# Ycblue/TransMIL-DeepGraft

Measured on AMD Instinct MI355X. Metric: slides/sec (fwd+bwd) at N=8192 patches, d=512, higher is better.
Workload: dtype bf16; 1 GPU; TransMIL_feat 2-class, 1 bag N=8192x512 per GPU, train step fwd+CE+bwd+allreduce+Lookahead(RAdam); execution=hipGraph replay of the whole step (one graph per resident bag), global_batch=1, seq_len=8192, parallelism=dp1, accumulate_grad_batches=1

## Files before the change

transmil_deepgraft_amd/csrc/pinv_split.hip:

```cpp
#include "common.h"
#include "a3_combine.h"
#include "../../include/transmil_hip.h"

namespace {

constexpr int NL = 256;
constexpr int MAT = NL * NL;
constexpr int PC = 64 * 128;
constexpr int SLOT = 4 * PC;
constexpr int NSLOT = 3;
constexpr int STAGE_LDS = NSLOT * SLOT;
constexpr int EROW = 68;
constexpr int EPI_LDS = 64 * EROW * 4;
constexpr int MAXJ = 3;
constexpr int NPROD = 8;
constexpr int NTHREADS = 64 * (4 + NPROD);

typedef __attribute__((address_space(3))) void lds_t;
typedef __attribute__((address_space(1))) void glb_t;
typedef __attribute__((address_space(3))) bf16x4 lds_v4;

struct SOp {
  const bf16* p;
  int kr;
  int pad;
};

enum { KIND_PRODUCT = 0, KIND_ABSSUMS = 1 };

struct SJob {
  SOp a[2], b[2];
  int nterms, kind;
  float alpha, diag;
  int alpha_cpow, e1_cpow;
  const void* e1; float e1s; int e1_f32;
  const void* e2; float e2s; int e2_f32;
  void* c; int c_f32; int pad0;
  float* cf;
  bf16* c2; float c2_alpha, c2_diag, c2_e1;
  bf16* c3; float c3_e1; int pad1;
};
TM_DEV const float* job_dotx(const SJob& J) { return (const float*)J.e2; }
TM_DEV float* job_dot_part(const SJob& J) { return J.cf; }

struct SLaunch {
  SJob j[MAXJ];
  int njobs, nbh;
  long long plane;
  const float* maxima;
  const float* X;
  float* sums;
  float* maxima_out;
  A3Combine a3;
#ifdef TM_DIAG
  unsigned long long* stamps;
#endif
};

#ifdef TM_DIAG
unsigned long long* g_split_stamps = nullptr;
#define SPLIT_STAMPS (stamp_out != nullptr)
#else
#define SPLIT_STAMPS false
#endif

TM_DEV unsigned long long stamp() {
  unsigned long long t;
  asm volatile("s_memtime %0\n\ts_waitcnt lgkmcnt(0)" : "=s"(t)::"memory");
  return t;
}
TM_DEV unsigned long long rstamp() {
  unsigned long long t;
  asm volatile("s_memrealtime %0\n\ts_waitcnt lgkmcnt(0)" : "=s"(t)::"memory");
  return t;
}

TM_DEV float powc(float c, int p) { return p == 0 ? 1.f : (p == 1 ? c : c * c); }

TM_DEV float inv_c(const float* maxima, int nbh) {
  typedef const __attribute__((address_space(4))) float cfloat;
  cfloat* m = (cfloat*)(uintptr_t)maxima;
  float mc = -INFINITY, mr = -INFINITY;
  for (int h = 0; h < nbh; ++h) { mc = fmaxf(mc, m[h]); mr = fmaxf(mr, m[nbh + h]); }
  return 1.f / (mc * mr);
}

TM_DEV unsigned lds_off(const void* p) { return (unsigned)(uintptr_t)(const __attribute__((address_space(3))) char*)p; }
template <int OFF> TM_DEV void ds_b128(bf16x8& d, unsigned a) {
  asm volatile("ds_read_b128 %0, %1 offset:%2" : "=v"(d) : "v"(a), "n"(OFF) : "memory");
}
template <int OFF> TM_DEV void ds_tr(bf16x4& d, unsigned a) {
  asm volatile("ds_read_b64_tr_b16 %0, %1 offset:%2" : "=v"(d) : "v"(a), "n"(OFF) : "memory");
}
template <int N> TM_DEV void wait_lgkm() {
  asm volatile("s_waitcnt lgkmcnt(%0)" ::"n"(N) : "memory");
  __builtin_amdgcn_sched_barrier(0);
}

TM_DEV unsigned kc_addr(int ob, int s, int lane) {
  const int r = ob + (lane & 31), c = 2 * s + (lane >> 5);
  return r * 128 + ((c ^ ((r >> 1) & 7)) << 4);
}
TM_DEV unsigned kr_addr(int ob, int lane) {
  const int g = lane >> 4, q = (lane & 15) >> 2, p = lane & 3;
  const int o = ob + (g & 1) * 16 + 4 * p;
  const int k = 8 * (g >> 1) + q;
  const int c = o >> 3, half = (o >> 2) & 1;
  return k * 128 + ((c ^ (((k >> 1) & 1) << 2)) << 4) + half * 8;
}

struct Frag { bf16x8 h, l; };
TM_DEV bf16x8 join(const bf16x4& a, const bf16x4& b) { return (bf16x8){a[0], a[1], a[2], a[3], b[0], b[1], b[2], b[3]}; }

template <int KR, int S, int PL>
TM_DEV void read_op(Frag& f, unsigned krbase, const unsigned (&kc)[4]) {
  if constexpr (KR) {
    bf16x4 a, b, c, d;
    ds_tr<PL * PC + S * 2048>(a, krbase);
    ds_tr<PL * PC + S * 2048 + 512>(b, krbase);
    ds_tr<(PL + 1) * PC + S * 2048>(c, krbase);
    ds_tr<(PL + 1) * PC + S * 2048 + 512>(d, krbase);
    f.h = join(a, b);
    f.l = join(c, d);
  } else {
    ds_b128<PL * PC>(f.h, kc[S]);
    ds_b128<(PL + 1) * PC>(f.l, kc[S]);
  }
}

template <int AKR, int BKR>
TM_DEV void chunk_mma(f32x16& acc, unsigned sb, unsigned akr, unsigned bkr, const unsigned (&akc0)[4],
                      const unsigned (&bkc0)[4]) {
  constexpr int RS = (AKR ? 4 : 2) + (BKR ? 4 : 2);
  unsigned akc[4], bkc[4];
#pragma unroll
  for (int s = 0; s < 4; ++s) { akc[s] = akc0[s] + sb; bkc[s] = bkc0[s] + sb; }
  const unsigned ab = akr + sb, bb = bkr + sb;
  Frag a[2], b[2];
  read_op<AKR, 0, 0>(a[0], ab, akc); read_op<BKR, 0, 2>(b[0], bb, bkc);
  read_op<AKR, 1, 0>(a[1], ab, akc); read_op<BKR, 1, 2>(b[1], bb, bkc);
  wait_lgkm<RS>();
  acc = __builtin_amdgcn_mfma_f32_32x32x16_bf16(a[0].l, b[0].h, acc, 0, 0, 0);
  acc = __builtin_amdgcn_mfma_f32_32x32x16_bf16(a[0].h, b[0].l, acc, 0, 0, 0);
  acc = __builtin_amdgcn_mfma_f32_32x32x16_bf16(a[0].h, b[0].h, acc, 0, 0, 0);
  read_op<AKR, 2, 0>(a[0], ab, akc); read_op<BKR, 2, 2>(b[0], bb, bkc);
  wait_lgkm<RS>();
  acc = __builtin_amdgcn_mfma_f32_32x32x16_bf16(a[1].l, b[1].h, acc, 0, 0, 0);
  acc = __builtin_amdgcn_mfma_f32_32x32x16_bf16(a[1].h, b[1].l, acc, 0, 0, 0);
  acc = __builtin_amdgcn_mfma_f32_32x32x16_bf16(a[1].h, b[1].h, acc, 0, 0, 0);
  read_op<AKR, 3, 0>(a[1], ab, akc); read_op<BKR, 3, 2>(b[1], bb, bkc);
  wait_lgkm<RS>();
  acc = __builtin_amdgcn_mfma_f32_32x32x16_bf16(a[0].l, b[0].h, acc, 0, 0, 0);
  acc = __builtin_amdgcn_mfma_f32_32x32x16_bf16(a[0].h, b[0].l, acc, 0, 0, 0);
  acc = __builtin_amdgcn_mfma_f32_32x32x16_bf16(a[0].h, b[0].h, acc, 0, 0, 0);
  wait_lgkm<0>();
  acc = __builtin_amdgcn_mfma_f32_32x32x16_bf16(a[1].l, b[1].h, acc, 0, 0, 0);
  acc = __builtin_amdgcn_mfma_f32_32x32x16_bf16(a[1].h, b[1].l, acc, 0, 0, 0);
  acc = __builtin_amdgcn_mfma_f32_32x32x16_bf16(a[1].h, b[1].h, acc, 0, 0, 0);
}

template <int N>
TM_DEV void wait_vm() { asm volatile("s_waitcnt vmcnt(%0)" ::"n"(N) : "memory"); }

TM_DEV void load_split8(const bf16* hi, long long plane, size_t off, float* v) {
  const bf16x8 h = *(const bf16x8*)(hi + off), l = *(const bf16x8*)(hi + plane + off);
#pragma unroll
  for (int e = 0; e < 8; ++e) v[e] = (float)h[e] + (float)l[e];
}
typedef unsigned u32x4_t __attribute__((ext_vector_type(4)));
TM_DEV void st16(void* base, size_t off_bytes, f32x4 v, bool wt) {
  if (wt)
    __builtin_amdgcn_raw_buffer_store_b128(__builtin_bit_cast(u32x4_t, v), tm_rsrc(base, 0x7FFFFFF0u),
                                           (unsigned)off_bytes, 0, 16);
  else
    *(f32x4*)((char*)base + off_bytes) = v;
}
TM_DEV void store_split8(bf16* hi, long long plane, size_t off, const float* v, bool wt = false) {
  bf16x8 h, l;
#pragma unroll
  for (int e = 0; e < 8; ++e) {
    h[e] = (bf16)v[e];
    l[e] = (bf16)(v[e] - (float)h[e]);
  }
  st16(hi, off * 2, __builtin_bit_cast(f32x4, h), wt);
  st16(hi, (plane + off) * 2, __builtin_bit_cast(f32x4, l), wt);
}
TM_DEV void load_f8(const float* p, size_t off, float* v) {
  const f32x4 a = *(const f32x4*)(p + off), b = *(const f32x4*)(p + off + 4);
  v[0] = a[0]; v[1] = a[1]; v[2] = a[2]; v[3] = a[3]; v[4] = b[0]; v[5] = b[1]; v[6] = b[2]; v[7] = b[3];
}
TM_DEV void store_f8(float* p, size_t off, const float* v, bool wt = false) {
  st16(p, off * 4, (f32x4){v[0], v[1], v[2], v[3]}, wt);
  st16(p, (off + 4) * 4, (f32x4){v[4], v[5], v[6], v[7]}, wt);
}

TM_DEV void abssums(const SLaunch& L, int head, int which, float* red) {
  const int t = threadIdx.x, lane = t & 63, wave = t >> 6;
  const bool on = t < NL;
  const float* x = L.X + (size_t)head * MAT;
  float s = 0.f;
  if (which == 0) {
    float* part = red + 16 + (wave & 3) * 64 * 65;
    if (on)
      for (int r = 0; r < 64; ++r) {
        const f32x4 v = *(const f32x4*)(x + (size_t)(wave * 64 + r) * NL + lane * 4);
        part[r * 65 + lane] = fabsf(v[0]) + fabsf(v[1]) + fabsf(v[2]) + fabsf(v[3]);
      }
    __syncthreads();
    if (on)
      for (int l = 0; l < 64; ++l) s += part[lane * 65 + l];
  } else if (on) {
    for (int i = 0; i < NL; ++i) s += fabsf(x[(size_t)i * NL + t]);
  }
  if (on) L.sums[((size_t)which * L.nbh + head) * NL + t] = s;
  const float m = wave_max(s);
  if (lane == 0 && on) red[wave] = m;
  __syncthreads();
  if (t == 0) L.maxima_out[which * L.nbh + head] = fmaxf(fmaxf(red[0], red[1]), fmaxf(red[2], red[3]));
}

template <bool DOT = false>
TM_DEV void stage_tile(const SJob& J, int nbh, long long plane, const float* maxima, int head, int tile,
                       char* smem, unsigned long long* stamp_out, bool dj = false) {
  const int tid = threadIdx.x, lane = tid & 63;
  const int wv = __builtin_amdgcn_readfirstlane(tid >> 6);
  const int m0 = (tile >> 2) * 64, n0 = (tile & 3) * 64;
  const size_t hoff = (size_t)head * MAT;
  const int nch = J.nterms * 4;
  const bool st_on = SPLIT_STAMPS;
  unsigned long long ts[8] = {0, 0, 0, 0, 0, 0, 0, 0};
  if (st_on) { ts[0] = rstamp(); ts[1] = stamp(); }

  const int lr = tid >> 3, lc = (tid & 7) * 8;
  const size_t eoff = hoff + (size_t)(m0 + lr) * NL + n0 + lc;
  const void* e1p = J.e1;
  const void* e2p = J.e2;
  const int e1f = J.e1_f32, e2f = J.e2_f32;
  f32x4 e1raw[2], e2raw[2];
  auto ld4 = [&](const f32x4* a) { return *a; };
  auto eload = [&](const void* e, int f32, f32x4 (&r)[2]) {
    if (f32) {
      const float* q = (const float*)e;
      r[0] = ld4((const f32x4*)(q + eoff)); r[1] = ld4((const f32x4*)(q + eoff + 4));
    } else {
      const bf16* q = (const bf16*)e;
      r[0] = ld4((const f32x4*)(q + eoff)); r[1] = ld4((const f32x4*)(q + plane + eoff));
    }
  };
  const bool epi = tid < 512;
  if (e1p && epi) eload(e1p, e1f, e1raw);
  const bool dotj = DOT && dj;
  if (!dotj && e2p && epi) eload(e2p, e2f, e2raw);
  float dxv[8];
  if (dotj && epi) {
    const float* dotx = job_dotx(J);
#pragma unroll
    for (int e = 0; e < 8; ++e) dxv[e] = dotx[hoff + (size_t)(n0 + lc + e) * NL + m0 + lr];
  }
  const bool need_c = J.alpha_cpow || J.e1_cpow;
  float mcv = -INFINITY, mrv = -INFINITY;
  if (need_c && nbh <= 64 && lane < nbh) { mcv = maxima[lane]; mrv = maxima[nbh + lane]; }
  float* ep = (float*)(smem + STAGE_LDS);

  if (wv >= 4) {
    constexpr int PPW = 32 / NPROD;
    const int p = wv - 4, pl = p / (NPROD / 4), rb = (p % (NPROD / 4)) * PPW * 8;
    const SOp op0 = pl < 2 ? J.a[0] : J.b[0];
    const SOp op1 = pl < 2 ? J.a[1] : J.b[1];
    const int o0w = pl < 2 ? m0 : n0;
    const bf16* const pb0 = op0.p + hoff + ((pl & 1) ? plane : 0);
    const bf16* const pb1 = op1.p + hoff + ((pl & 1) ? plane : 0);
    unsigned loff[2][PPW];
#pragma unroll
    for (int i = 0; i < PPW; ++i) {
      const int row = rb + i * 8 + (lane >> 3), pos = lane & 7;
      loff[0][i] = row * NL + 8 * (pos ^ ((row >> 1) & 7));
      loff[1][i] = row * NL + 8 * (pos ^ (((row >> 1) & 1) << 2));
    }
    auto issue = [&](int c) {
      char* img = smem + (c % NSLOT) * SLOT + pl * PC + rb * 128;
      const int t = c >> 2, k0 = (c & 3) * 64;
      const int kr = t ? op1.kr : op0.kr;
      const bf16* base = (t ? pb1 : pb0) + (kr ? k0 * NL + o0w : o0w * NL + k0);
#pragma unroll
      for (int i = 0; i < PPW; ++i)
        __builtin_amdgcn_global_load_lds((glb_t*)(base + (kr ? loff[1][i] : loff[0][i])), (lds_t*)(img + i * 1024),
                                         16, 0, 0);
    };
    issue(0);
    issue(1);
    for (int c = 0; c < nch; ++c) {
      if (c + 1 < nch) wait_vm<PPW>(); else wait_vm<0>();
      __builtin_amdgcn_s_barrier();
      asm volatile("" ::: "memory");
      if (c + 2 < nch) issue(c + 2);
    }
  } else {
    const int wm = wv >> 1, wn = wv & 1;
    const int code0 = J.a[0].kr | (J.b[0].kr << 1), code1 = J.a[1].kr | (J.b[1].kr << 1);
    const unsigned lbase = lds_off(smem);
    unsigned akc[4], bkc[4];
#pragma unroll
    for (int s = 0; s < 4; ++s) {
      akc[s] = lbase + kc_addr(wm * 32, s, lane);
      bkc[s] = lbase + kc_addr(wn * 32, s, lane);
    }
    const unsigned akr = lbase + kr_addr(wm * 32, lane), bkr = lbase + kr_addr(wn * 32, lane);
    f32x16 acc = (f32x16){};
    if (st_on) ts[2] = stamp();
    for (int c = 0; c < nch; ++c) {
      __builtin_amdgcn_s_barrier();
      asm volatile("" ::: "memory");
      if (st_on && c == 0) ts[3] = stamp();
      const unsigned sb = (c % NSLOT) * SLOT;
      switch ((c >> 2) ? code1 : code0) {
        case 0: chunk_mma<0, 0>(acc, sb, akr, bkr, akc, bkc); break;
        case 1: chunk_mma<1, 0>(acc, sb, akr, bkr, akc, bkc); break;
        case 2: chunk_mma<0, 1>(acc, sb, akr, bkr, akc, bkc); break;
        default: chunk_mma<1, 1>(acc, sb, akr, bkr, akc, bkc); break;
      }
      if (st_on && c == 0) ts[4] = stamp();
    }
    if (st_on) ts[5] = stamp();
    const int h = lane >> 5, cc = lane & 31;
#pragma unroll
    for (int r = 0; r < 16; ++r) ep[(wm * 32 + acc_row(r, h)) * EROW + wn * 32 + cc] = acc[r];
  }
  __syncthreads();
  __shared__ float dred[8];
  if (!epi) {
    if (dotj) __syncthreads();
    return;
  }
  const float diag = J.diag, e1s = J.e1s, e2s = J.e2s;
  float ic = 1.f;
  if (need_c) ic = nbh <= 64 ? 1.f / (wave_max(mcv) * wave_max(mrv)) : inv_c(maxima, nbh);
  const float alpha = J.alpha * powc(ic, J.alpha_cpow);
  const float e1m = powc(ic, J.e1_cpow);
  auto edecode = [&](const f32x4 (&r)[2], int f32, float* v) {
    if (f32) {
      const f32x4 x = r[0], y = r[1];
      v[0] = x[0]; v[1] = x[1]; v[2] = x[2]; v[3] = x[3]; v[4] = y[0]; v[5] = y[1]; v[6] = y[2]; v[7] = y[3];
    } else {
      const bf16x8 hh = __builtin_bit_cast(bf16x8, r[0]), ll = __builtin_bit_cast(bf16x8, r[1]);
#pragma unroll
      for (int e = 0; e < 8; ++e) v[e] = (float)hh[e] + (float)ll[e];
    }
  };
  {
    const int row = m0 + lr, col = n0 + lc;
    const bool dg = row >= col && row < col + 8;
    float s[8], e1v[8], e2v[8], v[8];
    {
      const f32x4 x0 = *(const f32x4*)(ep + lr * EROW + lc), x1 = *(const f32x4*)(ep + lr * EROW + lc + 4);
      s[0] = x0[0]; s[1] = x0[1]; s[2] = x0[2]; s[3] = x0[3]; s[4] = x1[0]; s[5] = x1[1]; s[6] = x1[2]; s[7] = x1[3];
    }
#pragma unroll
    for (int e = 0; e < 8; ++e) { s[e] *= alpha; e1v[e] = 0.f; e2v[e] = 0.f; }
    if (e1p) {
      edecode(e1raw, e1f, e1v);
#pragma unroll
      for (int e = 0; e < 8; ++e) e1v[e] *= e1m;
    }
    if (!dotj && e2p) edecode(e2raw, e2f, e2v);
#pragma unroll
    for (int e = 0; e < 8; ++e) v[e] = s[e] + e1s * e1v[e] + e2s * e2v[e];
    if (dg) v[row - col] += diag;
    const bool wt = true;
    if (J.c_f32) store_f8((float*)J.c, eoff, v, wt); else store_split8((bf16*)J.c, plane, eoff, v, wt);
    if (!dotj && J.cf) store_f8(J.cf, eoff, v, wt);
    if (J.c2) {
      float w[8];
      const float c2a = J.c2_alpha, c2e = J.c2_e1;
#pragma unroll
      for (int e = 0; e < 8; ++e) w[e] = c2a * s[e] + c2e * e1v[e];
      if (dg) w[row - col] += J.c2_diag;
      store_split8(J.c2, plane, eoff, w, wt);
    }
    if (J.c3) {
      float w[8];
      const float c3e = J.c3_e1;
#pragma unroll
      for (int e = 0; e < 8; ++e) w[e] = c3e * e1v[e];
      store_split8(J.c3, plane, eoff, w, wt);
    }
    if (dotj) {
      float d = 0.f;
#pragma unroll
      for (int e = 0; e < 8; ++e) d = fmaf(v[e], dxv[e], d);
      d = wave_sum(d);
      if (lane == 0) dred[wv] = d;
      __syncthreads();
      if (tid == 0)
        job_dot_part(J)[(size_t)head * 16 + tile] =
            ((dred[0] + dred[1]) + (dred[2] + dred[3])) + ((dred[4] + dred[5]) + (dred[6] + dred[7]));
    }
  }
  if (st_on && wv < 4) {
    ts[6] = stamp();
    ts[7] = rstamp();
    if (lane == 0) {
      unsigned long long* o = stamp_out + wv * 8;
#pragma unroll
      for (int i = 0; i < 8; ++i) o[i] = ts[i];
    }
  }
}

template <bool AUX, bool DOT = false>
__global__ __launch_bounds__(NTHREADS) void pinv_stage_kernel(SLaunch L) {
  extern __shared__ __attribute__((aligned(16))) char smem[];
  if (AUX && blockIdx.y == (unsigned)L.njobs) {
    A3CombineLds* lds = (A3CombineLds*)smem;
    const int g = threadIdx.x >> 8, t = threadIdx.x & 255;
    const int item = blockIdx.x * (NTHREADS / 256) + g;
    const bool active = item < L.a3.nbh * 32;
    const int bh = active ? item >> 5 : 0, qy = item & 31;
    const A3CombineState st = a3_combine_phase1(L.a3, bh, qy, t, lds[g], active);
    __syncthreads();
    a3_combine_phase2(L.a3, bh, qy, t, lds[g], st, active);
    return;
  }
  const SJob& J = L.j[blockIdx.y];
  const int u = blockIdx.x;
  const int nbh = L.nbh;
  const int head = u % nbh, tile = u / nbh;
  if (J.kind == KIND_ABSSUMS) {
    if (u < 2 * nbh) abssums(L, head, tile, (float*)smem);
    return;
  }
  unsigned long long* so = nullptr;
#ifdef TM_DIAG
  if (L.stamps) so = L.stamps + ((size_t)blockIdx.y * gridDim.x + blockIdx.x) * 4 * 8;
#endif
  stage_tile<DOT>(J, nbh, L.plane, L.maxima, head, tile, smem, so, DOT && (int)blockIdx.y == L.njobs - 1);
}

constexpr int APPLY_ROWS = 4;
constexpr int APPLY_SUMS = 8;
__global__ __launch_bounds__(256) void pinv_apply_bwd_kernel(const float* __restrict__ X, const float* __restrict__ sums,
                                                             const float* __restrict__ maxima, const bf16* __restrict__ G0,
                                                             long long plane, const float* __restrict__ part, int npart,
                                                             int nbh,
                                                             const float* __restrict__ dXc, int softmax,
                                                             float* __restrict__ out) {
  __shared__ float red[4][16];
  __shared__ float bc[4];
  constexpr int RB = APPLY_ROWS;
  const int bh = blockIdx.x, i0 = blockIdx.y * RB, t = threadIdx.x, lane = t & 63, wave = t >> 6;
  const size_t hb = (size_t)bh * MAT;
  static_assert(RB == 4 || RB == 8, "one 8- or 16-B piece per plane of G0's transposed row");
  float g0[RB], xv[RB], dx[RB];
  {
    const size_t o = hb + (size_t)t * NL + i0;
    if constexpr (RB == 8) {
      const bf16x8 h0 = *(const bf16x8*)(G0 + o), l0 = *(const bf16x8*)(G0 + plane + o);
#pragma unroll
      for (int e = 0; e < 8; ++e) g0[e] = (float)h0[e] + (float)l0[e];
    } else {
      const bf16x4 h0 = *(const bf16x4*)(G0 + o), l0 = *(const bf16x4*)(G0 + plane + o);
#pragma unroll
      for (int e = 0; e < 4; ++e) g0[e] = (float)h0[e] + (float)l0[e];
    }
  }
#pragma unroll
  for (int ii = 0; ii < RB; ++ii) {
    const size_t off = hb + (size_t)(i0 + ii) * NL + t;
    xv[ii] = X[off];
    dx[ii] = dXc[off];
  }
  const float* rs = sums + (size_t)bh * NL;
  const float* cs = sums + (size_t)(nbh + bh) * NL;
  const float csv = cs[t];
  float rsv[RB];
#pragma unroll
  for (int q = 0; q < RB / 4; ++q) {
    const f32x4 v = *(const f32x4*)(rs + i0 + 4 * q);
    rsv[4 * q] = v[0]; rsv[4 * q + 1] = v[1]; rsv[4 * q + 2] = v[2]; rsv[4 * q + 3] = v[3];
  }
  const int total = nbh * NL;
  float sc[APPLY_SUMS], sr[APPLY_SUMS];
#pragma unroll
  for (int u = 0; u < APPLY_SUMS; ++u) {
    const int e = min(t + 256 * u, total - 1);
    sc[u] = sums[e];
    sr[u] = sums[total + e];
  }
  const float mcl = lane < nbh ? maxima[lane] : -INFINITY, mrl = lane < nbh ? maxima[nbh + lane] : -INFINITY;
  float ps = t < npart ? part[t] : 0.f;
  float mc = wave_max(mcl), mr = wave_max(mrl);
  for (int h = 64; h < nbh; ++h) { mc = fmaxf(mc, maxima[h]); mr = fmaxf(mr, maxima[nbh + h]); }
  float nc = 0.f, nr = 0.f;
#pragma unroll
  for (int u = 0; u < APPLY_SUMS; ++u)
    if (t + 256 * u < total) { nc += sc[u] == mc; nr += sr[u] == mr; }
  for (int e = t + 256 * APPLY_SUMS; e < total; e += 256) { nc += sums[e] == mc; nr += sums[total + e] == mr; }
  for (int e = t + 256; e < npart; e += 256) ps += part[e];
  nc = wave_sum(nc); nr = wave_sum(nr); ps = wave_sum(ps);
  if (lane == 0) { red[wave][0] = nc; red[wave][1] = nr; red[wave][2] = ps; }
  __syncthreads();
  if (t == 0) {
    bc[0] = (red[0][0] + red[1][0]) + (red[2][0] + red[3][0]);
    bc[1] = (red[0][1] + red[1][1]) + (red[2][1] + red[3][1]);
    bc[2] = (red[0][2] + red[1][2]) + (red[2][2] + red[3][2]);
  }
  __syncthreads();
  const float c = mc * mr, ic = 1.f / c;
  const float dc = -bc[2] * ic * ic;
  const float dMc = dc * mr / bc[0], dMr = dc * mc / bc[1];
  const float tie_r = csv == mr ? dMr : 0.f;
#pragma unroll
  for (int ii = 0; ii < RB; ++ii) {
    const float sg = xv[ii] > 0.f ? 1.f : (xv[ii] < 0.f ? -1.f : 0.f);
    const float tie_c = rsv[ii] == mc ? dMc : 0.f;
    dx[ii] = dx[ii] + g0[ii] * ic + sg * (tie_c + tie_r);
  }
  if (!softmax) {
#pragma unroll
    for (int ii = 0; ii < RB; ++ii) out[hb + (size_t)(i0 + ii) * NL + t] = dx[ii];
    return;
  }
  __syncthreads();
#pragma unroll
  for (int ii = 0; ii < RB; ++ii) {
    const float d = wave_sum(xv[ii] * dx[ii]);
    if (lane == 0) red[wave][ii] = d;
  }
  __syncthreads();
#pragma unroll
  for (int ii = 0; ii < RB; ++ii) {
    const float rd = (red[0][ii] + red[1][ii]) + (red[2][ii] + red[3][ii]);
    out[hb + (size_t)(i0 + ii) * NL + t] = xv[ii] * (dx[ii] - rd);
  }
}

#define TM_HD __host__ __device__ inline

TM_HD SOp op(const void* p, int kr) { return SOp{(const bf16*)p, kr, 0}; }

TM_HD SJob product(SOp a, SOp b, void* c, float alpha, float diag = 0.f) {
  SJob j{};
  j.kind = KIND_PRODUCT;
  j.nterms = 1;
  j.a[0] = a; j.b[0] = b;
  j.c = c;
  j.alpha = alpha; j.diag = diag;
  return j;
}

struct FwdLayout {
  long long mat;
  int iters;
  float* base;
  TM_HD float* zf() const { return base; }
  TM_HD bf16* z(int k) const { return (bf16*)(base + (long long)k * mat); }
  TM_HD bf16* p(int k) const { return (bf16*)(base + (long long)(iters + 1 + k) * mat); }
  TM_HD bf16* t3(int k) const { return (bf16*)(base + (long long)(2 * iters + 1 + k) * mat); }
  TM_HD bf16* t5(int k) const { return (bf16*)(base + (long long)(3 * iters + 1 + k) * mat); }
  TM_HD bf16* scratch(int i) const { return (bf16*)(base + (long long)(4 * iters + 1 + i) * mat); }
  TM_HD float* sums() const { return base + (long long)(4 * iters + 3) * mat; }
  TM_HD float* maxima(int nbh) const { return sums() + 2LL * nbh * NL; }
};

TM_HD FwdLayout fwd_layout(float* saved, int nbh, int iters) {
  FwdLayout f;
  f.mat = (long long)nbh * MAT;
  f.iters = iters;
  f.base = saved;
  return f;
}

struct ChainArgs {
  const bf16* Xs;
  float* saved;
  float* work;
  int nbh, iters;
  const float* X = nullptr;
  float* part = nullptr;
};

TM_HD int fwd_levels(int iters) { return 2 * iters + 1; }
TM_HD int fwd_level_njobs(int iters, int lvl) {
  if (lvl == 2 * iters) return 1;
  const int k = lvl >> 1;
  return (lvl & 1) == 0 ? (k >= 1 ? 2 : 1) : (k + 1 < iters ? 2 : 1);
}
TM_HD SJob fwd_level_job(const ChainArgs& a, int lvl, int jn) {
  const FwdLayout F = fwd_layout(a.saved, a.nbh, a.iters);
  const int iters = a.iters;
  if (lvl == 2 * iters) {
    SJob z = iters == 1 ? product(op(a.Xs, 1), op(F.t5(0), 1), F.z(1), 0.25f)
                        : product(op(F.z(iters - 1), 0), op(F.t5(iters - 1), 1), F.z(iters), 0.25f);
    if (iters == 1) z.alpha_cpow = 1;
    z.cf = F.zf();
    return z;
  }
  const int k = lvl >> 1;
  bf16* R = F.scratch((k + 1) & 1);
  if ((lvl & 1) == 0) {
    if (jn == 0) {
      SJob r;
      if (k == 0) {
        r = product(op(F.scratch(0), 0), op(F.scratch(0), 1), R, 1.f);
        r.alpha_cpow = 2;
        r.e1 = F.scratch(0); r.e1_cpow = 1;
        r.c3 = F.p(0); r.c3_e1 = 1.f;
      } else {
        r = product(op(F.p(k), 0), op(F.p(k), 1), R, 1.f);
        r.e1 = F.p(k);
      }
      r.c2 = F.t3(k); r.c2_alpha = 1.f; r.c2_diag = 15.f; r.c2_e1 = -7.f;
      return r;
    }
    SJob z = k == 1 ? product(op(a.Xs, 1), op(F.t5(0), 1), F.z(1), 0.25f)
                    : product(op(F.z(k - 1), 0), op(F.t5(k - 1), 1), F.z(k), 0.25f);
    if (k == 1) z.alpha_cpow = 1;
    return z;
  }
  if (jn == 0) return product(op(F.p(k), 0), op(F.t3(k), 1), F.t5(k), -1.f, 13.f);
  SJob p = product(op(R, 0), op(F.t3(k), 1), F.p(k + 1), -0.25f);
  p.e1 = F.p(k); p.e1s = 3.25f;
  return p;
}

TM_HD int bwd_levels(int iters) { return 4 * iters; }
TM_HD int bwd_level_njobs(int iters, int lvl) { return (lvl & 3) == 2 ? 1 : 2; }
TM_HD SJob bwd_level_job(const ChainArgs& a, int lvl, int jn) {
  const FwdLayout F = fwd_layout(a.saved, a.nbh, a.iters);
  const long long mat = F.mat;
  float* work = a.work;
  bf16* G = (bf16*)work;
  bf16* dT5 = (bf16*)(work + mat);
  bf16* dZa = (bf16*)(work + 2 * mat);
  bf16* dP = (bf16*)(work + 3 * mat);
  bf16* dT3 = (bf16*)(work + 4 * mat);
  float* dXc = work + 5 * mat;
  const int k = a.iters - 1 - (lvl >> 2);
  switch (lvl & 3) {
    case 0:
      if (jn == 0) {
        SJob j = k == 0 ? product(op(a.Xs, 0), op(G, 1), dT5, 0.25f)
                        : product(op(F.z(k), 1), op(G, 1), dT5, 0.25f);
        if (k == 0) j.alpha_cpow = 1;
        return j;
      }
      return product(op(G, 0), op(F.t5(k), 0), dZa, 0.25f);
    case 1:
      if (jn == 0) return product(op(dT5, 0), op(F.t3(k), 0), dP, -1.f);
      return product(op(F.p(k), 1), op(dT5, 1), dT3, -1.f);
    case 2: {
      SJob j = product(op(dT3, 0), op(F.p(k), 0), dP, 1.f);
      j.nterms = 2;
      j.a[1] = op(F.p(k), 1); j.b[1] = op(dT3, 1);
      j.e1 = dP; j.e1s = 1.f;
      j.e2 = dT3; j.e2s = -7.f;
      return j;
    }
    default:
      if (jn == 0) {
        SJob j = k == 0 ? product(op(dP, 0), op(a.Xs, 1), dXc, 1.f)
                        : product(op(dP, 0), op(F.z(k), 0), dXc, 1.f);
        if (k == 0) j.alpha_cpow = 1;
        j.c_f32 = 1;
        if (k != a.iters - 1) { j.e1 = dXc; j.e1_f32 = 1; j.e1s = 1.f; }
        return j;
      }
      SJob g = product(op(a.Xs, 1), op(dP, 1), G, 1.f);
      g.e1 = dZa; g.e1s = 1.f;
      if (k == 0 && a.X) { g.e2 = a.X; g.cf = a.part; }
      return g;
  }
}

struct Launcher {
  SLaunch L{};
  explicit Launcher(int nbh, long long plane, const float* maxima) {
    L.nbh = nbh; L.plane = plane; L.maxima = maxima;
#ifdef TM_DIAG
    L.stamps = g_split_stamps;
#endif
  }
  bool dot = false;
  void add(const SJob& j) { L.j[L.njobs++] = j; }
  int go(hipStream_t st) {
    dim3 grid(16 * L.nbh, L.njobs);
    if (L.a3.w) {
      grid.y += 1;
      tm_allow_smem(pinv_stage_kernel<true>, STAGE_LDS + EPI_LDS);
      pinv_stage_kernel<true><<<grid, NTHREADS, STAGE_LDS + EPI_LDS, st>>>(L);
    } else if (dot) {
      tm_allow_smem(pinv_stage_kernel<false, true>, STAGE_LDS + EPI_LDS);
      pinv_stage_kernel<false, true><<<grid, NTHREADS, STAGE_LDS + EPI_LDS, st>>>(L);
    } else {
      tm_allow_smem(pinv_stage_kernel<false>, STAGE_LDS + EPI_LDS);
      pinv_stage_kernel<false><<<grid, NTHREADS, STAGE_LDS + EPI_LDS, st>>>(L);
    }
    TM_CHECK_LAUNCH();
#ifdef TM_DIAG
    if (g_split_stamps) g_split_stamps += (size_t)grid.x * grid.y * 4 * 8;
#endif
    return 0;
  }
};

int run_levels(const ChainArgs& c, int dir, long long plane, const float* maxima, hipStream_t st,
               const A3Combine* a3 = nullptr) {
  const int nlev = dir == 0 ? fwd_levels(c.iters) : bwd_levels(c.iters);
  for (int lvl = 0; lvl < nlev; ++lvl) {
    Launcher l(c.nbh, plane, maxima);
    const int nj = dir == 0 ? fwd_level_njobs(c.iters, lvl) : bwd_level_njobs(c.iters, lvl);
    for (int j = 0; j < nj; ++j) l.add(dir == 0 ? fwd_level_job(c, lvl, j) : bwd_level_job(c, lvl, j));
    l.dot = dir == 1 && lvl == nlev - 1 && c.X != nullptr;
    if (a3 && dir == 0 && lvl == nlev - 1) l.L.a3 = *a3;
    if (int rc = l.go(st)) return rc;
  }
  return 0;
}

}

extern "C" long long tm_pinv_split_saved_floats(int nbh, int iters) {
  return (4LL * iters + 3) * nbh * MAT + 2LL * nbh * NL + 2LL * nbh;
}

int pinv_fwd_split(const float* X, const void* Xs, int nbh, int iters, float* saved, const A3Combine* a3,
                   void* stream);

extern "C" int tm_pinv_fwd_split(const float* X, const void* Xs, int nbh, int iters, float* saved, void* stream) {
  return pinv_fwd_split(X, Xs, nbh, iters, saved, nullptr, stream);
}

extern "C" int tm_pinv_fwd_split_a3(const float* X, const void* Xs, int nbh, int iters, float* saved,
                                    const float* a3_work, int a3_parts, float* w, float* lse3, void* stream) {
  TM_REQUIRE(a3_work && w && lse3 && a3_parts >= 1, "pinv_fwd_split_a3: bad A3 args");
  const bf16* po = (const bf16*)a3_work;
  const float* pm = a3_work + (size_t)a3_parts * nbh * NL * 64;
  const float* pl = pm + (size_t)a3_parts * nbh * NL;
  const A3Combine a3{po, pm, pl, a3_parts, nbh, w, lse3};
  return pinv_fwd_split(X, Xs, nbh, iters, saved, &a3, stream);
}

int pinv_fwd_split(const float* X, const void* Xs, int nbh, int iters, float* saved, const A3Combine* a3,
                   void* stream) {
  TM_REQUIRE(X && Xs && saved && nbh > 0 && iters >= 1, "pinv_fwd_split: bad args (iters >= 1)");
  TM_REQUIRE(((uintptr_t)Xs % 16) == 0 && ((uintptr_t)saved % 16) == 0, "pinv_fwd_split: 16-B aligned buffers");
  hipStream_t st = (hipStream_t)stream;
  const FwdLayout F = fwd_layout(saved, nbh, iters);
  const long long plane = F.mat;
  float* maxima = F.maxima(nbh);
  {
    Launcher l(nbh, plane, nullptr);
    l.add(product(op(Xs, 0), op(Xs, 0), F.scratch(0), 1.f));
    SJob s{};
    s.kind = KIND_ABSSUMS;
    l.add(s);
    l.L.X = X; l.L.sums = F.sums(); l.L.maxima_out = maxima;
    if (int rc = l.go(st)) return rc;
  }
  const ChainArgs c{(const bf16*)Xs, saved, nullptr, nbh, iters};
  return run_levels(c, 0, plane, maxima, st, a3);
}

extern "C" long long tm_pinv_bwd_split_workspace_floats(int nbh) {
  return 6LL * nbh * MAT + nbh * 16LL + 64;
}

extern "C" int tm_pinv_bwd_split(const float* X, const void* Xs, int nbh, int iters, const float* saved, float* work,
                                 int softmax, float* out, void* stream) {
  TM_REQUIRE(X && Xs && saved && work && out && nbh > 0 && iters >= 1, "pinv_bwd_split: bad args");
  hipStream_t st = (hipStream_t)stream;
  const FwdLayout F = fwd_layout((float*)saved, nbh, iters);
  const long long mat = F.mat, plane = mat;
  const float* maxima = F.maxima(nbh);
  bf16* G = (bf16*)work;
  float* dXc = work + 5 * mat;
  float* part = work + 6 * mat;
  ChainArgs c{(const bf16*)Xs, (float*)saved, work, nbh, iters};
  c.X = X;
  c.part = part;
  if (int rc = run_levels(c, 1, plane, maxima, st)) return rc;
  pinv_apply_bwd_kernel<<<dim3(nbh, NL / APPLY_ROWS), 256, 0, st>>>(X, F.sums(), maxima, G, plane, part, nbh * 16, nbh, dXc,
                                                        softmax, out);
  TM_CHECK_LAUNCH();
  return 0;
}

#ifdef TM_DIAG
extern "C" void tm_debug_set_split_stamps(unsigned long long* buf) { g_split_stamps = buf; }
#endif

__global__ void split_kernel(const float* __restrict__ x, bf16* __restrict__ y, long long count) {
  const long long i = ((long long)blockIdx.x * 256 + threadIdx.x) * 8;
  if (i >= count) return;
  float v[8];
  load_f8(x, i, v);
  store_split8(y, count, i, v);
}

extern "C" int tm_split_f32(const float* x, void* y, long long count, void* stream) {
  TM_REQUIRE(count % 8 == 0 && ((uintptr_t)x % 16) == 0 && ((uintptr_t)y % 16) == 0, "split_f32: count % 8, alignment");
  if (count == 0) return 0;
  split_kernel<<<(unsigned)((count / 8 + 255) / 256), 256, 0, (hipStream_t)stream>>>(x, (bf16*)y, count);
  TM_CHECK_LAUNCH();
  return 0;
}
```

Baseline: 933.6 slides/sec.

## Speed pinv stage kernel prologue with bulk scalar kernarg loads and early addend loads

Changes the pinv stage kernel prologue so each block loads its 192-byte SJob and the launch scalars with a few wide s_load_dwordx16/x8 instructions. Per-lane LDS addresses are computed while those loads are in flight. The grid becomes 3-D (head, tile, job), which removes the divide and modulo. Epilogue addend loads (e1/e2, dot operand, maxima) are moved so they issue after the first producer fetch or at the start of the consumer waves, with explicit global address-space casts. The aim is to shorten per-block startup latency, at the cost of hand-written asm and layout static_asserts that make the code fragile.

After: 956.4 slides/sec, median of 6. 2.4% higher.

```diff
diff --git a/transmil_deepgraft_amd/csrc/pinv_split.hip b/transmil_deepgraft_amd/csrc/pinv_split.hip
--- a/transmil_deepgraft_amd/csrc/pinv_split.hip
+++ b/transmil_deepgraft_amd/csrc/pinv_split.hip
@@ -28,7 +28,7 @@
 
 enum { KIND_PRODUCT = 0, KIND_ABSSUMS = 1 };
 
-struct SJob {
+struct alignas(64) SJob {
   SOp a[2], b[2];
   int nterms, kind;
   float alpha, diag;
@@ -40,6 +40,7 @@
   bf16* c2; float c2_alpha, c2_diag, c2_e1;
   bf16* c3; float c3_e1; int pad1;
 };
+static_assert(sizeof(SJob) == 192, "SJob: three 64-B lines");
 TM_DEV const float* job_dotx(const SJob& J) { return (const float*)J.e2; }
 TM_DEV float* job_dot_part(const SJob& J) { return J.cf; }
 
@@ -74,6 +75,12 @@
   asm volatile("s_memrealtime %0\n\ts_waitcnt lgkmcnt(0)" : "=s"(t)::"memory");
   return t;
 }
+
+typedef unsigned u32x2_t __attribute__((ext_vector_type(2)));
+typedef unsigned u32x4_t __attribute__((ext_vector_type(4)));
+typedef unsigned u32x8_t __attribute__((ext_vector_type(8)));
+typedef unsigned u32x16_t __attribute__((ext_vector_type(16)));
+template <class T> TM_DEV T* as_global(T* p) { return (T*)(__attribute__((address_space(1))) T*)p; }
 
 TM_DEV float powc(float c, int p) { return p == 0 ? 1.f : (p == 1 ? c : c * c); }
 
@@ -167,7 +174,6 @@
 #pragma unroll
   for (int e = 0; e < 8; ++e) v[e] = (float)h[e] + (float)l[e];
 }
-typedef unsigned u32x4_t __attribute__((ext_vector_type(4)));
 TM_DEV void st16(void* base, size_t off_bytes, f32x4 v, bool wt) {
   if (wt)
     __builtin_amdgcn_raw_buffer_store_b128(__builtin_bit_cast(u32x4_t, v), tm_rsrc(base, 0x7FFFFFF0u),
@@ -219,17 +225,44 @@
   if (t == 0) L.maxima_out[which * L.nbh + head] = fmaxf(fmaxf(red[0], red[1]), fmaxf(red[2], red[3]));
 }
 
+constexpr int PPW = 32 / NPROD;
+constexpr int NPRE = 10;
+static_assert(2 * PPW <= NPRE, "pre[] holds a producer's offsets");
+TM_DEV void lane_addresses(int wv, int lane, const char* smem, unsigned (&pre)[NPRE]) {
+  if (wv >= 4) {
+    const int rb = ((wv - 4) % (NPROD / 4)) * PPW * 8;
+#pragma unroll
+    for (int i = 0; i < PPW; ++i) {
+      const int row = rb + i * 8 + (lane >> 3), pos = lane & 7;
+      pre[i] = row * NL + 8 * (pos ^ ((row >> 1) & 7));
+      pre[PPW + i] = row * NL + 8 * (pos ^ (((row >> 1) & 1) << 2));
+    }
+#pragma unroll
+    for (int i = 2 * PPW; i < NPRE; ++i) pre[i] = 0;
+  } else {
+    const int wm = wv >> 1, wn = wv & 1;
+    const unsigned lbase = lds_off(smem);
+#pragma unroll
+    for (int s = 0; s < 4; ++s) {
+      pre[s] = lbase + kc_addr(wm * 32, s, lane);
+      pre[4 + s] = lbase + kc_addr(wn * 32, s, lane);
+    }
+    pre[8] = lbase + kr_addr(wm * 32, lane);
+    pre[9] = lbase + kr_addr(wn * 32, lane);
+  }
+}
+
 template <bool DOT = false>
 TM_DEV void stage_tile(const SJob& J, int nbh, long long plane, const float* maxima, int head, int tile,
-                       char* smem, unsigned long long* stamp_out, bool dj = false) {
+                       char* smem, const unsigned (&pre)[NPRE], unsigned long long* stamp_out, unsigned long long t0,
+                       unsigned long long t1, bool dj = false) {
   const int tid = threadIdx.x, lane = tid & 63;
   const int wv = __builtin_amdgcn_readfirstlane(tid >> 6);
   const int m0 = (tile >> 2) * 64, n0 = (tile & 3) * 64;
   const size_t hoff = (size_t)head * MAT;
   const int nch = J.nterms * 4;
   const bool st_on = SPLIT_STAMPS;
-  unsigned long long ts[8] = {0, 0, 0, 0, 0, 0, 0, 0};
-  if (st_on) { ts[0] = rstamp(); ts[1] = stamp(); }
+  unsigned long long ts[8] = {t0, t1, 0, 0, 0, 0, 0, 0};
 
   const int lr = tid >> 3, lc = (tid & 7) * 8;
   const size_t eoff = hoff + (size_t)(m0 + lr) * NL + n0 + lc;
@@ -237,7 +270,9 @@
   const void* e2p = J.e2;
   const int e1f = J.e1_f32, e2f = J.e2_f32;
   f32x4 e1raw[2], e2raw[2];
-  auto ld4 = [&](const f32x4* a) { return *a; };
+  typedef const __attribute__((address_space(1))) f32x4 gf32x4;
+  typedef const __attribute__((address_space(1))) float gfloat;
+  auto ld4 = [&](const f32x4* a) { return *(gf32x4*)a; };
   auto eload = [&](const void* e, int f32, f32x4 (&r)[2]) {
     if (f32) {
       const float* q = (const float*)e;
@@ -247,23 +282,25 @@
       r[0] = ld4((const f32x4*)(q + eoff)); r[1] = ld4((const f32x4*)(q + plane + eoff));
     }
   };
-  const bool epi = tid < 512;
-  if (e1p && epi) eload(e1p, e1f, e1raw);
+  const bool epi = wv < 8;
   const bool dotj = DOT && dj;
-  if (!dotj && e2p && epi) eload(e2p, e2f, e2raw);
   float dxv[8];
-  if (dotj && epi) {
-    const float* dotx = job_dotx(J);
-#pragma unroll
-    for (int e = 0; e < 8; ++e) dxv[e] = dotx[hoff + (size_t)(n0 + lc + e) * NL + m0 + lr];
-  }
   const bool need_c = J.alpha_cpow || J.e1_cpow;
   float mcv = -INFINITY, mrv = -INFINITY;
-  if (need_c && nbh <= 64 && lane < nbh) { mcv = maxima[lane]; mrv = maxima[nbh + lane]; }
+  asm volatile("" : "+v"(mcv), "+v"(mrv));
+  auto load_addends = [&]() {
+    if (e1p) eload(e1p, e1f, e1raw);
+    if (!dotj && e2p) eload(e2p, e2f, e2raw);
+    if (dotj) {
+      const float* dotx = job_dotx(J);
+#pragma unroll
+      for (int e = 0; e < 8; ++e) dxv[e] = *(gfloat*)(dotx + hoff + (size_t)(n0 + lc + e) * NL + m0 + lr);
+    }
+    if (need_c && nbh <= 64 && lane < nbh) { mcv = *(gfloat*)(maxima + lane); mrv = *(gfloat*)(maxima + nbh + lane); }
+  };
   float* ep = (float*)(smem + STAGE_LDS);
 
   if (wv >= 4) {
-    constexpr int PPW = 32 / NPROD;
     const int p = wv - 4, pl = p / (NPROD / 4), rb = (p % (NPROD / 4)) * PPW * 8;
     const SOp op0 = pl < 2 ? J.a[0] : J.b[0];
     const SOp op1 = pl < 2 ? J.a[1] : J.b[1];
@@ -272,11 +309,7 @@
     const bf16* const pb1 = op1.p + hoff + ((pl & 1) ? plane : 0);
     unsigned loff[2][PPW];
 #pragma unroll
-    for (int i = 0; i < PPW; ++i) {
-      const int row = rb + i * 8 + (lane >> 3), pos = lane & 7;
-      loff[0][i] = row * NL + 8 * (pos ^ ((row >> 1) & 7));
-      loff[1][i] = row * NL + 8 * (pos ^ (((row >> 1) & 1) << 2));
-    }
+    for (int i = 0; i < PPW; ++i) { loff[0][i] = pre[i]; loff[1][i] = pre[PPW + i]; }
     auto issue = [&](int c) {
       char* img = smem + (c % NSLOT) * SLOT + pl * PC + rb * 128;
       const int t = c >> 2, k0 = (c & 3) * 64;
@@ -288,6 +321,9 @@
                                          16, 0, 0);
     };
     issue(0);
+    __builtin_amdgcn_sched_barrier(0);
+    if (epi) load_addends();
+    __builtin_amdgcn_sched_barrier(0);
     issue(1);
     for (int c = 0; c < nch; ++c) {
       if (c + 1 < nch) wait_vm<PPW>(); else wait_vm<0>();
@@ -296,16 +332,13 @@
       if (c + 2 < nch) issue(c + 2);
     }
   } else {
+    load_addends();
     const int wm = wv >> 1, wn = wv & 1;
     const int code0 = J.a[0].kr | (J.b[0].kr << 1), code1 = J.a[1].kr | (J.b[1].kr << 1);
-    const unsigned lbase = lds_off(smem);
     unsigned akc[4], bkc[4];
 #pragma unroll
-    for (int s = 0; s < 4; ++s) {
-      akc[s] = lbase + kc_addr(wm * 32, s, lane);
-      bkc[s] = lbase + kc_addr(wn * 32, s, lane);
-    }
-    const unsigned akr = lbase + kr_addr(wm * 32, lane), bkr = lbase + kr_addr(wn * 32, lane);
+    for (int s = 0; s < 4; ++s) { akc[s] = pre[s]; bkc[s] = pre[4 + s]; }
+    const unsigned akr = pre[8], bkr = pre[9];
     f32x16 acc = (f32x16){};
     if (st_on) ts[2] = stamp();
     for (int c = 0; c < nch; ++c) {
@@ -392,7 +425,7 @@
       if (lane == 0) dred[wv] = d;
       __syncthreads();
       if (tid == 0)
-        job_dot_part(J)[(size_t)head * 16 + tile] =
+        *(__attribute__((address_space(1))) float*)(job_dot_part(J) + (size_t)head * 16 + tile) =
             ((dred[0] + dred[1]) + (dred[2] + dred[3])) + ((dred[4] + dred[5]) + (dred[6] + dred[7]));
     }
   }
@@ -410,10 +443,50 @@
 template <bool AUX, bool DOT = false>
 __global__ __launch_bounds__(NTHREADS) void pinv_stage_kernel(SLaunch L) {
   extern __shared__ __attribute__((aligned(16))) char smem[];
-  if (AUX && blockIdx.y == (unsigned)L.njobs) {
+  unsigned long long t0 = 0, t1 = 0;
+#ifdef TM_DIAG
+  t0 = rstamp(); t1 = stamp();
+#endif
+  static_assert(offsetof(SLaunch, j) == 0 && offsetof(SLaunch, njobs) == MAXJ * sizeof(SJob), "SLaunch layout");
+  static_assert(offsetof(SLaunch, nbh) == offsetof(SLaunch, njobs) + 4 && offsetof(SLaunch, plane) == offsetof(SLaunch, njobs) + 8 &&
+                offsetof(SLaunch, maxima) == offsetof(SLaunch, njobs) + 16, "SLaunch scalars: one 8-dword load");
+  struct Raw { u32x16_t l[3]; };
+  static_assert(sizeof(Raw) == sizeof(SJob), "SJob: three 16-dword loads");
+  Raw raw;
+  u32x8_t rs;
+  {
+    typedef const __attribute__((address_space(4))) char kchar;
+    kchar* kp = (kchar*)__builtin_amdgcn_kernarg_segment_ptr();
+    kchar* jp = kp + (size_t)min((int)blockIdx.z, MAXJ - 1) * sizeof(SJob);
+    asm volatile("s_load_dwordx16 %0, %4, 0x0\n\ts_load_dwordx16 %1, %4, 0x40\n\ts_load_dwordx16 %2, %4, 0x80\n\t"
+                 "s_load_dwordx8 %3, %5, %6"
+                 : "=&s"(raw.l[0]), "=&s"(raw.l[1]), "=&s"(raw.l[2]), "=&s"(rs)
+                 : "s"(jp), "s"(kp), "n"(MAXJ * sizeof(SJob)));
+  }
+  unsigned pre[NPRE];
+  lane_addresses(__builtin_amdgcn_readfirstlane(threadIdx.x >> 6), threadIdx.x & 63, smem, pre);
+  {
+    u32x4_t pa = {pre[0], pre[1], pre[2], pre[3]}, pb = {pre[4], pre[5], pre[6], pre[7]};
+    u32x2_t pc = {pre[8], pre[9]};
+    asm volatile("s_waitcnt lgkmcnt(0)"
+                 : "+s"(raw.l[0]), "+s"(raw.l[1]), "+s"(raw.l[2]), "+s"(rs), "+v"(pa), "+v"(pb), "+v"(pc));
+#pragma unroll
+    for (int i = 0; i < 4; ++i) { pre[i] = pa[i]; pre[4 + i] = pb[i]; }
+    pre[8] = pc[0]; pre[9] = pc[1];
+  }
+  SJob J = __builtin_bit_cast(SJob, raw);
+  const int njobs = (int)rs[0], nbh = (int)rs[1];
+  const long long plane = (long long)(((unsigned long long)rs[3] << 32) | rs[2]);
+  const float* maxima = as_global((const float*)(((unsigned long long)rs[5] << 32) | rs[4]));
+  for (int t = 0; t < 2; ++t) { J.a[t].p = as_global(J.a[t].p); J.b[t].p = as_global(J.b[t].p); }
+  J.e1 = as_global(J.e1); J.e2 = as_global(J.e2); J.c = as_global(J.c); J.cf = as_global(J.cf);
+  J.c2 = as_global(J.c2); J.c3 = as_global(J.c3);
+  const int head = blockIdx.x, tile = blockIdx.y;
+  const int u = tile * nbh + head;
+  if (AUX && blockIdx.z == (unsigned)njobs) {
     A3CombineLds* lds = (A3CombineLds*)smem;
     const int g = threadIdx.x >> 8, t = threadIdx.x & 255;
-    const int item = blockIdx.x * (NTHREADS / 256) + g;
+    const int item = u * (NTHREADS / 256) + g;
     const bool active = item < L.a3.nbh * 32;
     const int bh = active ? item >> 5 : 0, qy = item & 31;
     const A3CombineState st = a3_combine_phase1(L.a3, bh, qy, t, lds[g], active);
@@ -421,19 +494,15 @@
     a3_combine_phase2(L.a3, bh, qy, t, lds[g], st, active);
     return;
   }
-  const SJob& J = L.j[blockIdx.y];
-  const int u = blockIdx.x;
-  const int nbh = L.nbh;
-  const int head = u % nbh, tile = u / nbh;
   if (J.kind == KIND_ABSSUMS) {
-    if (u < 2 * nbh) abssums(L, head, tile, (float*)smem);
+    if (tile < 2) abssums(L, head, tile, (float*)smem);
     return;
   }
   unsigned long long* so = nullptr;
 #ifdef TM_DIAG
-  if (L.stamps) so = L.stamps + ((size_t)blockIdx.y * gridDim.x + blockIdx.x) * 4 * 8;
+  if (L.stamps) so = L.stamps + ((size_t)blockIdx.z * 16 * nbh + u) * 4 * 8;
 #endif
-  stage_tile<DOT>(J, nbh, L.plane, L.maxima, head, tile, smem, so, DOT && (int)blockIdx.y == L.njobs - 1);
+  stage_tile<DOT>(J, nbh, plane, maxima, head, tile, smem, pre, so, t0, t1, DOT && (int)blockIdx.z == njobs - 1);
 }
 
 constexpr int APPLY_ROWS = 4;
@@ -683,9 +752,9 @@
   bool dot = false;
   void add(const SJob& j) { L.j[L.njobs++] = j; }
   int go(hipStream_t st) {
-    dim3 grid(16 * L.nbh, L.njobs);
+    dim3 grid(L.nbh, 16, L.njobs);
     if (L.a3.w) {
-      grid.y += 1;
+      grid.z += 1;
       tm_allow_smem(pinv_stage_kernel<true>, STAGE_LDS + EPI_LDS);
       pinv_stage_kernel<true><<<grid, NTHREADS, STAGE_LDS + EPI_LDS, st>>>(L);
     } else if (dot) {
@@ -697,7 +766,7 @@
     }
     TM_CHECK_LAUNCH();
 #ifdef TM_DIAG
-    if (g_split_stamps) g_split_stamps += (size_t)grid.x * grid.y * 4 * 8;
+    if (g_split_stamps) g_split_stamps += (size_t)grid.x * grid.y * grid.z * 4 * 8;
 #endif
     return 0;
   }
```
